# ShuangXieIrene/ssds.pytorch

Measured on AMD Instinct MI355X. Metric: images/sec (fwd+decode+NMS) SSD-MobileNetV2@512, higher is better.
Workload: dtype bf16

## Files before the change

### ssds.pytorch_amd/csrc/ssdk_mbflow.hip

```cpp
#include <stdio.h>
#include <atomic>
#include <type_traits>

#include "ssdk_common.h"
#include "ssdk_flow_common.h"

namespace ssdk {

constexpr int kFlowThreads = 256;

template <int NCH, int NFO>
struct FlowLds {
  static constexpr int T = (NCH + 1) / 2;
  static constexpr int we = 0;
  static constexpr int sb = we + NCH * 1024;
  static constexpr int wd = sb + NCH * 4 * 32;
  static constexpr int bd = wd + NCH * 9 * 4 * 8;
  static constexpr int wp = (bd + NCH * 4 * 8 + 15) & ~15;
  static constexpr int spb = wp + NFO * T * 1024;
  static constexpr int bytes = spb + NFO * 4 * 32;
};

template <int DT, int S, int NCH, int NFO, int NS, bool STEM = false, bool YE = false, bool PAIR = false, bool XD = false>
__global__ __launch_bounds__(kFlowThreads, ((STEM && !YE) || PAIR) ? 3 : 2) void mbflow_kernel(const FlowParams p) {
// ... 383 lines not shown
              db[s][3] = 0u;
            }
          }
#pragma unroll
          for (int f = 0; f < NFO; ++f) {
            const u32x4 wf = *reinterpret_cast<const u32x4*>(smem + L::wp + ((f * T + t) * 64 + (int)lane) * 16);
#pragma unroll
            for (int s = 0; s < NA; ++s) yacc[s][f] = fl_mfma<SSDK_F16>(wf, db[s], yacc[s][f]);
          }
        }
#pragma unroll
        for (int s = 0; s < NA; ++s) {
          if (out_lane[s]) {
            u16* yrow = p.y + (((size_t)n * p.Ho + oy_fin) * p.Wo + oxl[s]) * Cout;
#pragma unroll
            for (int f = 0; f < NFO; ++f) {
              const int co = f * 16 + (int)fg * 4;
              if (co < Cout) {
                const f32x4 spv = *reinterpret_cast<const f32x4*>(smem + L::spb + (f * 4 + (int)fg) * 32);
                const f32x4 bpv = *reinterpret_cast<const f32x4*>(smem + L::spb + (f * 4 + (int)fg) * 32 + 16);
                u32 h01 = fl_pack2<DT>(fmaf(yacc[s][f][0], spv[0], bpv[0]), fmaf(yacc[s][f][1], spv[1], bpv[1]));
                u32 h23 = fl_pack2<DT>(fmaf(yacc[s][f][2], spv[2], bpv[2]), fmaf(yacc[s][f][3], spv[3], bpv[3]));
                if (!STEM && !MERGE && p.residual) {
                  const u32 x01 = resv[s][f].x, x23 = resv[s][f].y;
                  h01 = fl_pack2<DT>(fl_from16<DT>(h01 & 0xffffu) + fl_from16<DT>(x01 & 0xffffu), fl_from16<DT>(h01 >> 16) + fl_from16<DT>(x01 >> 16));
                  h23 = fl_pack2<DT>(fl_from16<DT>(h23 & 0xffffu) + fl_from16<DT>(x23 & 0xffffu), fl_from16<DT>(h23 >> 16) + fl_from16<DT>(x23 >> 16));
                }
                *reinterpret_cast<uint2*>(yrow + co) = make_uint2(h01, h23);
              }
            }
          }
        }
      }
    }
    if (dbgw && dbg_k < 250) p.dbg[dbg_k++] = __builtin_readcyclecounter();
  };


  auto row2 = [&](const XRow (&x0)[NS], const XRow (&x1)[NS], int iy, fl_h2 (&a0)[NA][NCH * 2], fl_h2 (&a1)[NA][NCH * 2],
                  fl_h2 (&a2)[NA][NCH * 2], fl_h2 (&a3)[NA][NCH * 2]) {
    if (dbgw && dbg_k < 250) {
      p.dbg[dbg_k++] = __builtin_readcyclecounter();
      asm volatile("s_waitcnt vmcnt(4)" ::: "memory");
      p.dbg[dbg_k++] = __builtin_readcyclecounter();
    }
    u32x4 xf[2][NS];
    fl_f2 hi[2][NS];
#pragma unroll
    for (int s = 0; s < NS; ++s) {
#pragma unroll
      for (int q = 0; q < 4; ++q) {
        xf[0][s][q] = x0[s].w[q];
        xf[1][s][q] = x1[s].w[q];
      }
      const float k0 = (col_ok[s] && (unsigned)iy < (unsigned)p.H) ? kFlSixth : 0.f;
      const float k1 = (col_ok[s] && (unsigned)(iy + 1) < (unsigned)p.H) ? kFlSixth : 0.f;
      hi[0][s] = fl_f2{k0, k0};
      hi[1][s] = fl_f2{k1, k1};
    }
    const bool st[2] = {iy - 1 >= oy0 && iy - 1 <= oy1, iy >= oy0 && iy <= oy1};
    uint2 resv[2][NA][NFO];
    if (p.residual) {
#pragma unroll
      for (int o = 0; o < 2; ++o)
#pragma unroll
        for (int s = 0; s < NA; ++s)
#pragma unroll
          for (int f = 0; f < NFO; ++f) {
            const int co = f * 16 + (int)fg * 4;
            uint2 r = make_uint2(0u, 0u);
            if (st[o] && out_lane[s] && co < Cout) r = *reinterpret_cast<const uint2*>(ximg + ((size_t)(iy - 1 + o) * p.W + oxl[s]) * Cin + co);
            resv[o][s][f] = r;
          }
    }
    asm volatile("" ::: "memory");
    f32x4 e_cur[2][NS], e_nxt[2][NS];
    u32x4 wa = *reinterpret_cast<const u32x4*>(smem + L::we + (int)lane * 16);
    {
      const f32x4 bv0 = *reinterpret_cast<const f32x4*>(smem + L::sb + (int)fg * 32 + 16);
#pragma unroll
      for (int o = 0; o < 2; ++o)
#pragma unroll
        for (int s = 0; s < NS; ++s) e_cur[o][s] = fl_mfma<DT>(wa, xf[o][s], bv0);
    }
    if (NCH > 1) wa = *reinterpret_cast<const u32x4*>(smem + L::we + (64 + (int)lane) * 16);
#pragma unroll
    for (int c = 0; c < NCH; ++c) {
      asm volatile("" ::: "memory");
      uint2 wt[9];
#pragma unroll
      for (int t = 0; t < 9; ++t) wt[t] = *reinterpret_cast<const uint2*>(smem + L::wd + ((c * 9 + t) * 4 + (int)fg) * 8);
      const uint2 bdi = *reinterpret_cast<const uint2*>(smem + L::bd + (c * 4 + (int)fg) * 8);
      if (c + 1 < NCH) {
        const f32x4 bvn = *reinterpret_cast<const f32x4*>(smem + L::sb + ((c + 1) * 4 + (int)fg) * 32 + 16);
#pragma unroll
        for (int o = 0; o < 2; ++o)
#pragma unroll
          for (int s = 0; s < NS; ++s) e_nxt[o][s] = fl_mfma<DT>(wa, xf[o][s], bvn);
        if (c + 2 < NCH) wa = *reinterpret_cast<const u32x4*>(smem + L::we + ((c + 2) * 64 + (int)lane) * 16);
      }
      __builtin_amdgcn_sched_barrier(0);
      auto taps = [&](int ky, fl_h2 l0, fl_h2 l1, fl_h2 c0, fl_h2 c1, fl_h2 r0, fl_h2 r1, fl_h2& q0, fl_h2& q1) {
        const uint2 w0 = wt[ky * 3], w1 = wt[ky * 3 + 1], w2 = wt[ky * 3 + 2];
        fl_h2 s0 = ky == 0 ? fl_as_h2(bdi.x) : q0, s1 = ky == 0 ? fl_as_h2(bdi.y) : q1;
        s0 = __builtin_elementwise_fma(l0, fl_as_h2(w0.x), s0);
        s1 = __builtin_elementwise_fma(l1, fl_as_h2(w0.y), s1);
        s0 = __builtin_elementwise_fma(c0, fl_as_h2(w1.x), s0);
        s1 = __builtin_elementwise_fma(c1, fl_as_h2(w1.y), s1);
        if (ky == 2) {
          s0 = fl_fma_clamp01(r0, fl_as_h2(w2.x), s0);
          s1 = fl_fma_clamp01(r1, fl_as_h2(w2.y), s1);
        } else {
          s0 = __builtin_elementwise_fma(r0, fl_as_h2(w2.x), s0);
          s1 = __builtin_elementwise_fma(r1, fl_as_h2(w2.y), s1);
        }
        asm volatile("" : "+v"(s0), "+v"(s1));
        q0 = s0;
        q1 = s1;
      };
#pragma unroll
      for (int o = 0; o < 2; ++o) {
#pragma unroll
        for (int s = 0; s < NS; ++s) {
          const f32x4 e = e_cur[o][s];
          const u32 w0 = fl_unit_pack(e[0], e[1], hi[o][s]), w1 = fl_unit_pack(e[2], e[3], hi[o][s]);
          const fl_h2 l0 = fl_as_h2(fl_from_left(w0)), l1 = fl_as_h2(fl_from_left(w1)), c0 = fl_as_h2(w0), c1 = fl_as_h2(w1);
          const fl_h2 r0 = fl_as_h2(fl_from_right(w0)), r1 = fl_as_h2(fl_from_right(w1));
          if (o == 0) {
            taps(0, l0, l1, c0, c1, r0, r1, a2[s][2 * c], a2[s][2 * c + 1]);
            taps(1, l0, l1, c0, c1, r0, r1, a1[s][2 * c], a1[s][2 * c + 1]);
            taps(2, l0, l1, c0, c1, r0, r1, a0[s][2 * c], a0[s][2 * c + 1]);
          } else {
            taps(0, l0, l1, c0, c1, r0, r1, a3[s][2 * c], a3[s][2 * c + 1]);
            taps(1, l0, l1, c0, c1, r0, r1, a2[s][2 * c], a2[s][2 * c + 1]);
            taps(2, l0, l1, c0, c1, r0, r1, a1[s][2 * c], a1[s][2 * c + 1]);
          }
        }
      }
#pragma unroll
      for (int o = 0; o < 2; ++o)
#pragma unroll
        for (int s = 0; s < NS; ++s) e_cur[o][s] = e_nxt[o][s];
      __builtin_amdgcn_sched_barrier(0);
    }
    if (dbgw && dbg_k < 250) p.dbg[dbg_k++] = __builtin_readcyclecounter();
    if (st[0] || st[1]) {
      asm volatile("" ::: "memory");
      f32x4 yacc[2][NA][NFO];
#pragma unroll
      for (int o = 0; o < 2; ++o)
#pragma unroll
        for (int s = 0; s < NA; ++s)
#pragma unroll
          for (int f = 0; f < NFO; ++f) yacc[o][s][f] = f32x4{0.f, 0.f, 0.f, 0.f};
#pragma unroll
      for (int t = 0; t < T; ++t) {
        u32x4 db[2][NA];
#pragma unroll
        for (int o = 0; o < 2; ++o)
#pragma unroll
          for (int s = 0; s < NA; ++s) {
            const fl_h2* fin = o == 0 ? a0[s] : a1[s];
            db[o][s][0] = fl_as_u32(fin[4 * t]);
            db[o][s][1] = fl_as_u32(fin[4 * t + 1]);
            if (2 * t + 1 < NCH) {
              db[o][s][2] = fl_as_u32(fin[(4 * t + 2 < NCH * 2) ? 4 * t + 2 : 0]);
              db[o][s][3] = fl_as_u32(fin[(4 * t + 3 < NCH * 2) ? 4 * t + 3 : 0]);
            } else {
              db[o][s][2] = 0u;
              db[o][s][3] = 0u;
            }
          }
#pragma unroll
        for (int f = 0; f < NFO; ++f) {
          const u32x4 wf = *reinterpret_cast<const u32x4*>(smem + L::wp + ((f * T + t) * 64 + (int)lane) * 16);
#pragma unroll
          for (int o = 0; o < 2; ++o)
#pragma unroll
            for (int s = 0; s < NA; ++s) yacc[o][s][f] = fl_mfma<SSDK_F16>(wf, db[o][s], yacc[o][s][f]);
        }
      }
#pragma unroll
      for (int f = 0; f < NFO; ++f) {
        const int co = f * 16 + (int)fg * 4;
        if (co < Cout) {
          const f32x4 spv = *reinterpret_cast<const f32x4*>(smem + L::spb + (f * 4 + (int)fg) * 32);
          const f32x4 bpv = *reinterpret_cast<const f32x4*>(smem + L::spb + (f * 4 + (int)fg) * 32 + 16);
#pragma unroll
          for (int o = 0; o < 2; ++o)
#pragma unroll
            for (int s = 0; s < NA; ++s) {
              if (!(st[o] && out_lane[s])) continue;
              u16* yrow = p.y + (((size_t)n * p.Ho + (iy - 1 + o)) * p.Wo + oxl[s]) * Cout;
              u32 h01 = fl_pack2<DT>(fmaf(yacc[o][s][f][0], spv[0], bpv[0]), fmaf(yacc[o][s][f][1], spv[1], bpv[1]));
              u32 h23 = fl_pack2<DT>(fmaf(yacc[o][s][f][2], spv[2], bpv[2]), fmaf(yacc[o][s][f][3], spv[3], bpv[3]));
              if (p.residual) {
                const u32 x01 = resv[o][s][f].x, x23 = resv[o][s][f].y;
                h01 = fl_pack2<DT>(fl_from16<DT>(h01 & 0xffffu) + fl_from16<DT>(x01 & 0xffffu), fl_from16<DT>(h01 >> 16) + fl_from16<DT>(x01 >> 16));
                h23 = fl_pack2<DT>(fl_from16<DT>(h23 & 0xffffu) + fl_from16<DT>(x23 & 0xffffu), fl_from16<DT>(h23 >> 16) + fl_from16<DT>(x23 >> 16));
              }
              *reinterpret_cast<uint2*>(yrow + co) = make_uint2(h01, h23);
            }
        }
      }
    }
    if (dbgw && dbg_k < 250) p.dbg[dbg_k++] = __builtin_readcyclecounter();
  };

  const auto Y = std::true_type{};
  const auto No = std::false_type{};
  auto load_row = [&](XRow (&dst)[NS], int iy) {
#pragma unroll
    for (int s = 0; s < NS; ++s) dst[s] = load_x(iy, s);
  };
  XRow xa[NS], xb[NS];
  {
    if constexpr (PAIR) {
      const int rend = oy1 + 1;
      XRow xc[NS], xd[NS];
      load_row(xa, oy0 - 1);
      load_row(xb, oy0);
      for (int r = oy0 - 1; r <= rend; r += 4) {
        load_row(xc, r + 2);
        load_row(xd, r + 3);
        row2(xa, xb, r, accA, accB, accC, accD);
        load_row(xa, r + 4);
        load_row(xb, r + 5);
        row2(xc, xd, r + 2, accC, accD, accA, accB);
      }
    } else if constexpr (S == 1) {
      const int rend = oy1 + 1;
      load_row(xa, oy0 - 1);
      for (int r = oy0 - 1; r <= rend; r += 6) {
        load_row(xb, r + 1);
        row(xa, r, Y, Y, Y, accA, accB, accC, r - 1);
        load_row(xa, r + 2);
        row(xb, r + 1, Y, Y, Y, accB, accC, accA, r);
        load_row(xb, r + 3);
        row(xa, r + 2, Y, Y, Y, accC, accA, accB, r + 1);
        load_row(xa, r + 4);
        row(xb, r + 3, Y, Y, Y, accA, accB, accC, r + 2);
        load_row(xb, r + 5);
        row(xa, r + 4, Y, Y, Y, accB, accC, accA, r + 3);
        load_row(xa, r + 6);
        row(xb, r + 5, Y, Y, Y, accC, accA, accB, r + 4);
      }
    } else {
      const int rend = 2 * oy1 + 1;
      load_row(xa, 2 * oy0 - 1);
      for (int r = 2 * oy0 - 1; r <= rend; r += 4) {
        load_row(xb, r + 1);
        row(xa, r, Y, No, Y, accA, accC, accB, (r - 1) / 2);
        load_row(xa, r + 2);
        row(xb, r + 1, No, Y, No, accC, accB, accC, 0);
        load_row(xb, r + 3);
        row(xa, r + 2, Y, No, Y, accB, accC, accA, (r + 1) / 2);
        load_row(xa, r + 4);
        row(xb, r + 3, No, Y, No, accC, accA, accC, 0);
      }
    }
  }
}

constexpr int kFlowNS = 2;

template <int DT, int S, int NCH, int NFO>
static void flow_launch(const FlowParams& p, unsigned grid, hipStream_t stream) {
  constexpr int lds = FlowLds<NCH, NFO>::bytes;
  if constexpr (S == 1 && NCH == 9) {
    if (p.layout == 101) {
      static const int pair = getenv("SSDK_FLOW_PAIR") ? atoi(getenv("SSDK_FLOW_PAIR")) : 1;
      if (pair) {
        (void)hipFuncSetAttribute(reinterpret_cast<const void*>(&mbflow_kernel<DT, S, NCH, NFO, 1, false, false, true>), hipFuncAttributeMaxDynamicSharedMemorySize, lds);
        hipLaunchKernelGGL((mbflow_kernel<DT, S, NCH, NFO, 1, false, false, true>), dim3(grid), dim3(kFlowThreads), lds, stream, p);
        return;
      }
      (void)hipFuncSetAttribute(reinterpret_cast<const void*>(&mbflow_kernel<DT, S, NCH, NFO, 1>), hipFuncAttributeMaxDynamicSharedMemorySize, lds);
      hipLaunchKernelGGL((mbflow_kernel<DT, S, NCH, NFO, 1>), dim3(grid), dim3(kFlowThreads), lds, stream, p);
      return;
    }
  }
  (void)hipFuncSetAttribute(reinterpret_cast<const void*>(&mbflow_kernel<DT, S, NCH, NFO, kFlowNS>), hipFuncAttributeMaxDynamicSharedMemorySize, lds);
  hipLaunchKernelGGL((mbflow_kernel<DT, S, NCH, NFO, kFlowNS>), dim3(grid), dim3(kFlowThreads), lds, stream, p);
}

template <int DT, int S>
static bool flow_dispatch(const FlowParams& p, int nch, int nfo, unsigned grid, hipStream_t stream) {
#define SSDK_FLOW(NCH_, NFO_)                                   \
  if (nch == NCH_ && nfo == NFO_) {                             \
    flow_launch<DT, S, NCH_, NFO_>(p, grid, stream);            \
    return true;                                                \
  }
  SSDK_FLOW(6, 2)
  SSDK_FLOW(9, 2)
  SSDK_FLOW(12, 2)
  SSDK_FLOW(12, 4)
#undef SSDK_FLOW
  return false;
}

int launch_mbflow(const ssdk_mbconv_desc* d, hipStream_t stream) {
  static const int env = getenv("SSDK_MB_FLOW") ? atoi(getenv("SSDK_MB_FLOW")) : 1;
  const int variant = d->variant;
  if ((!env && variant <= 0) || variant < 0 || variant == 2 || variant == 3) return 1;
  const bool stem = d->stem != 0;
  if (stem) {
    if (d->Cin > 3 || d->Chid != 32 || d->Cout != 16 || d->stride != 1 || d->residual) return 1;
  } else if (d->Cin > 32 || (d->Cin % 8) || d->Chid > 192 || (d->Chid % 16) || d->Cout > 64 || (d->Cout % 8)) {
    return 1;
  }
  const int nch = d->Chid / 16, nfo = stem ? 1 : (d->Cout <= 32 ? 2 : 4);
  if (!stem && !((nch == 6 || nch == 9 || nch == 12) && (nfo == 2 || nch == 12))) return 1;
  FlowParams p;
  p.x = (const u16*)d->x;
  p.y = (u16*)d->y;
  p.we = (const u16*)d->w_expand;
  p.se = d->scale_expand;
  p.be = d->bias_expand;
  p.wd = (const u16*)d->w_dw;
  p.bd = (const u16*)d->bias_dw;
  p.wp = (const u16*)d->w_project;
  p.sp = d->scale_project;
  p.bp = d->bias_project;
  p.N = d->N;
  p.H = d->H;
  p.W = d->W;
  p.Cin = d->Cin;
  p.Himg = d->H;
  p.Wimg = d->W;
  p.Cimg = d->Cin;
  p.layout = d->stem;
  if (stem) {
    p.H = (d->H + 2 - 3) / 2 + 1;
    p.W = (d->W + 2 - 3) / 2 + 1;
    p.Cin = 32;
  }
  p.Chid = d->Chid;
  p.Cout = d->Cout;
  p.Ho = (p.H + 2 - 3) / d->stride + 1;
  p.Wo = (p.W + 2 - 3) / d->stride + 1;
  p.residual = d->residual;
  p.seg_mask = 0;
  p.dbg = nullptr;
  static const int env_dbg = getenv("SSDK_MB_DBG") ? atoi(getenv("SSDK_MB_DBG")) : 0;
  static unsigned long long* dbg_dev = nullptr;
  if (env_dbg) {
    if (!dbg_dev) (void)hipMalloc(&dbg_dev, 256 * sizeof(unsigned long long));
    (void)hipMemsetAsync(dbg_dev, 0, 256 * sizeof(unsigned long long), stream);
    p.dbg = dbg_dev;
  }
  auto dbg_print = [&]() {
    if (!env_dbg) return;
    unsigned long long hh[256];
    (void)hipStreamSynchronize(stream);
    (void)hipMemcpy(hh, dbg_dev, sizeof(hh), hipMemcpyDeviceToHost);
    fprintf(stderr, "[mbflow dbg] Cin=%d Chid=%d Cout=%d s=%d stem=%d rs=%d: per row (wait x | chunks | project+store | to next row):", d->Cin,
            d->Chid, d->Cout, d->stride, (int)stem, p.rs);
    for (int i = 0; i + 4 < 250 && hh[i + 4]; i += 4)
      fprintf(stderr, " [%llu %llu %llu %llu]", hh[i + 1] - hh[i], hh[i + 2] - hh[i + 1], hh[i + 3] - hh[i + 2], hh[i + 4] - hh[i + 3]);
    fprintf(stderr, "\n");
  };
  const int ow = d->stride == 1 ? 14 : 7;
  p.strips = (p.Wo + ow - 1) / ow;
  if (d->stride == 2) p.strips = 2 * ((p.Wo + 14) / 15);
  constexpr int env_rs = 0;
  constexpr int env_ns1 = 1;
  const bool ns1 = ((env_ns1 & 1) && !stem && d->stride == 1 && nch == 9) || ((env_ns1 & 2) && stem);
  const int flow_ns = ns1 ? 1 : kFlowNS;
  if (ns1 && !stem) p.layout = 101;
  const int groups = (p.strips + flow_ns - 1) / flow_ns;
  int rs = 64;
  while (rs > 16 && (long)d->N * groups * ((p.Ho + rs - 1) / rs) < 4096) rs >>= 1;
  if ((long)d->N * groups * ((p.Ho + rs - 1) / rs) < 2048 && env_rs <= 0 && variant <= 0) return 1;
  if (variant > 0) {
    while (rs > 8 && (long)d->N * groups * ((p.Ho + rs - 1) / rs) < 2048) rs >>= 1;
  }
  if (env_rs > 0) rs = env_rs;
  if (rs > p.Ho) rs = p.Ho;
  p.rs = rs;
  p.segs = (p.Ho + rs - 1) / rs;
  const long items = (long)d->N * groups * p.segs;
  const unsigned grid = (unsigned)((items + 3) / 4);
  bool ok;
  if (stem) {
    if (p.segs > 64) return 1;
    unsigned long long edge = 0;
    for (int sgi = 0; sgi < p.segs; ++sgi) {
      const int o0 = sgi * p.rs, o1 = (o0 + p.rs < p.Ho ? o0 + p.rs : p.Ho) - 1;
      const int last_row = o1 + 1 < p.H - 1 ? o1 + 1 : p.H - 1;
      if (2 * last_row + 1 >= p.Himg) edge |= 1ull << sgi;
    }
    const unsigned long long all = p.segs == 64 ? ~0ull : ((1ull << p.segs) - 1ull);
    constexpr int lds = FlowLds<2, 1>::bytes;
    auto go = [&](auto DTc, auto YEc, unsigned long long mask) {
      constexpr int DTv = decltype(DTc)::value;
      constexpr bool YEv = decltype(YEc)::value;
      if (!mask) return;
      FlowParams q = p;
      q.seg_mask = mask;
      const long it = (long)d->N * groups * __builtin_popcountll(mask);
      const unsigned g = (unsigned)((it + 3) / 4);
      if (ns1) {
        (void)hipFuncSetAttribute(reinterpret_cast<const void*>(&mbflow_kernel<DTv, 1, 2, 1, 1, true, YEv>),
                                  hipFuncAttributeMaxDynamicSharedMemorySize, lds);
        hipLaunchKernelGGL((mbflow_kernel<DTv, 1, 2, 1, 1, true, YEv>), dim3(g), dim3(kFlowThreads), lds, stream, q);
        return;
      }
      if constexpr (!YEv) {
        static const int env_xd = getenv("SSDK_STEM_DWORD") ? atoi(getenv("SSDK_STEM_DWORD")) : 1;
        if (env_xd && q.layout == 1 && (q.Wimg & 1) == 0 && (reinterpret_cast<uintptr_t>(q.x) & 3u) == 0) {
          (void)hipFuncSetAttribute(reinterpret_cast<const void*>(&mbflow_kernel<DTv, 1, 2, 1, kFlowNS, true, false, false, true>),
                                    hipFuncAttributeMaxDynamicSharedMemorySize, lds);
          hipLaunchKernelGGL((mbflow_kernel<DTv, 1, 2, 1, kFlowNS, true, false, false, true>), dim3(g), dim3(kFlowThreads), lds, stream, q);
          return;
        }
      }
      (void)hipFuncSetAttribute(reinterpret_cast<const void*>(&mbflow_kernel<DTv, 1, 2, 1, kFlowNS, true, YEv>),
                                hipFuncAttributeMaxDynamicSharedMemorySize, lds);
      hipLaunchKernelGGL((mbflow_kernel<DTv, 1, 2, 1, kFlowNS, true, YEv>), dim3(g), dim3(kFlowThreads), lds, stream, q);
    };
    if (d->dtype == SSDK_BF16) {
      go(std::integral_constant<int, SSDK_BF16>{}, std::false_type{}, all & ~edge);
      go(std::integral_constant<int, SSDK_BF16>{}, std::true_type{}, edge);
    } else {
      go(std::integral_constant<int, SSDK_F16>{}, std::false_type{}, all & ~edge);
      go(std::integral_constant<int, SSDK_F16>{}, std::true_type{}, edge);
    }
    dbg_print();
    return 0;
  }
  if (d->dtype == SSDK_BF16) ok = d->stride == 1 ? flow_dispatch<SSDK_BF16, 1>(p, nch, nfo, grid, stream) : flow_dispatch<SSDK_BF16, 2>(p, nch, nfo, grid, stream);
  else ok = d->stride == 1 ? flow_dispatch<SSDK_F16, 1>(p, nch, nfo, grid, stream) : flow_dispatch<SSDK_F16, 2>(p, nch, nfo, grid, stream);
  if (ok) dbg_print();
  return ok ? 0 : 1;
}

}
```

### ssds.pytorch_amd/csrc/ssdk_mbk.hip

```cpp
#include "ssdk_common.h"
#include "ssdk_flow_common.h"
#include "ssdk_scan.h"

namespace ssdk {

struct MbkParams {
  const u16* x;
  u16* y;
  const unsigned char* img;
  int N, H, W, Ho, Wo, Cin, Chid, Cout, residual;
  int pairs, halves;
  unsigned items;
  unsigned long long* dbg;
  unsigned wave_mask, pair_mask;
};

template <int KS, int NW, int NCHW, int NFO>
struct MbkGeo {
  static constexpr int NP = (NCHW + 1) / 2;
  static constexpr int PAIR_KB = 2 * KS + NFO;
  static constexpr int MISC_KB = (NCHW * 384 + 1023) / 1024;
  static constexpr int m_be = 0, m_wd = NCHW * 64, m_bd = NCHW * (64 + 288);
  static constexpr int SPB_KB = 2;
  static_assert(NFO * 128 <= SPB_KB * 1024, "projection BN block");
  __host__ __device__ static size_t weights(int halves) { return (size_t)halves * NW * NP * PAIR_KB * 1024; }
  __host__ __device__ static size_t misc_off(int halves) { return weights(halves); }
  __host__ __device__ static size_t spb_off(int halves) { return misc_off(halves) + (size_t)NW * MISC_KB * 1024; }
  __host__ __device__ static size_t bytes(int halves) { return spb_off(halves) + (size_t)halves * SPB_KB * 1024; }
};

template <int S, int NS>
struct MbkItem {
  static constexpr int NXS = NS * S;
  static constexpr int NR = S + 3;
};

template <int S, int NS, int KS, int NW, int NCHW, int NFO>
struct MbkLds {
  using G = MbkGeo<KS, NW, NCHW, NFO>;
  using I = MbkItem<S, NS>;
  static constexpr int FT = 2 * NS * NFO;
  static constexpr int XF = FT % 5 == 0 ? 5 : (FT % 8 == 0 ? 8 : 4);
  static_assert(FT % XF == 0, "exchange rounds");
  static constexpr int xt = 0;
  static constexpr int misc = xt + I::NR * I::NXS * KS * 1024;
  static constexpr int spb = misc + NW * G::MISC_KB * 1024;
  static constexpr int xch = spb + G::SPB_KB * 1024;
  static constexpr int bytes = xch + NW * XF * 1024;
};

__device__ __forceinline__ void mbk_mfma_guard() {
  __builtin_amdgcn_sched_barrier(0);
  asm volatile("s_nop 15\n\ts_nop 3" ::: "memory");
  __builtin_amdgcn_sched_barrier(0);
}
__device__ __forceinline__ void mbk_valu_guard() {
  __builtin_amdgcn_sched_barrier(0);
  asm volatile("s_nop 3" ::: "memory");
  __builtin_amdgcn_sched_barrier(0);
}
__device__ __forceinline__ u32 fl_from_left2(u32 cur, u32 prev) {
  const int old = __builtin_amdgcn_update_dpp(0, (int)prev, 0x121, 0xf, 0xf, true);
  return (u32)__builtin_amdgcn_update_dpp(old, (int)cur, 0x111, 0xf, 0xf, false);
}
__device__ __forceinline__ u32 fl_from_right2(u32 cur, u32 next) {
  const int old = __builtin_amdgcn_update_dpp(0, (int)next, 0x12f, 0xf, 0xf, true);
  return (u32)__builtin_amdgcn_update_dpp(old, (int)cur, 0x101, 0xf, 0xf, false);
}

template <int DT, int S, int NS, int KS, int NW, int NCHW, int NFO, bool DBG = false>
__global__ __launch_bounds__(64 * NW, 2) void mbk_kernel(const MbkParams p) {
  using L = MbkLds<S, NS, KS, NW, NCHW, NFO>;
  using G = MbkGeo<KS, NW, NCHW, NFO>;
  using I = MbkItem<S, NS>;
  constexpr int NR = I::NR, NXS = I::NXS, NE = NR * NXS;
  constexpr int XF = L::XF, FT = L::FT, NP = G::NP, PAIR_KB = G::PAIR_KB;
  constexpr int NO = 2 * NS;
  constexpr bool ODD = (NCHW & 1) != 0;
  constexpr int ROUNDS = FT / XF;
  extern __shared__ __attribute__((aligned(16))) unsigned char smem[];
  const u32 tid = threadIdx.x, lane = tid & 63u;
  const u32 fr = lane & 15u, fg = lane >> 4;
  const int wv = __builtin_amdgcn_readfirstlane((int)(tid >> 6));
  const int Cin = p.Cin, Cout = p.Cout, H = p.H, W = p.W, Ho = p.Ho, Wo = p.Wo;

  const u32 item = blockIdx.x;
  const int half = (int)(item % (u32)p.halves);
  const u32 rem = item / (u32)p.halves;
  const int n = (int)(rem / (u32)p.pairs), rp = (int)(rem % (u32)p.pairs);
  const int oy0 = 2 * rp;
  const int iy0 = S * oy0 - 1;
  const int co_base = half * 16 * NFO;
  const u16* ximg = p.x + (size_t)n * H * W * Cin;
  const bool stamp = p.dbg != nullptr && blockIdx.x == 0 && tid == 0;
  if (stamp) p.dbg[0] = __builtin_readcyclecounter();

  const u32x4* wimg = reinterpret_cast<const u32x4*>(p.img + ((size_t)(half * NW + wv) * NP) * ((size_t)PAIR_KB * 1024)) + lane;
  u32x4 wa[KS], wb[KS];
#pragma unroll
  for (int ks = 0; ks < KS; ++ks) {
    wa[ks] = wimg[(size_t)ks * 64];
    wb[ks] = wimg[(size_t)(KS + ks) * 64];
  }

  for (int e = wv; e < NE; e += NW) {
    const int r = e / NXS, xs = e % NXS;
    int iy = iy0 + r;
    iy = iy < 0 ? 0 : (iy > H - 1 ? H - 1 : iy);
    const int col = S == 1 ? 16 * xs + (int)fr : 2 * (16 * (xs >> 1) + (int)fr) + (xs & 1);
    const u16* src = ximg + ((size_t)iy * W + col) * Cin + fg * 8;
#pragma unroll
    for (int ks = 0; ks < KS; ++ks)
      __builtin_amdgcn_global_load_lds((glb_u8*)(src + ks * 32), (lds_u8*)(smem + L::xt + (e * KS + ks) * 1024), 16, 0, 0);
  }
  {
    const unsigned char* src = p.img + G::misc_off(p.halves) + (size_t)wv * (G::MISC_KB * 1024) + lane * 16;
#pragma unroll
    for (int k = 0; k < G::MISC_KB; ++k)
      __builtin_amdgcn_global_load_lds((glb_u8*)(src + k * 1024), (lds_u8*)(smem + L::misc + (wv * G::MISC_KB + k) * 1024), 16, 0, 0);
  }
  if (wv == 0) {
    const unsigned char* src = p.img + G::spb_off(p.halves) + (size_t)half * (G::SPB_KB * 1024) + lane * 16;
#pragma unroll
    for (int k = 0; k < G::SPB_KB; ++k)
      __builtin_amdgcn_global_load_lds((glb_u8*)(src + k * 1024), (lds_u8*)(smem + L::spb + k * 1024), 16, 0, 0);
  }
  asm volatile("s_waitcnt vmcnt(0)" ::: "memory");
  __syncthreads();
  if (stamp) p.dbg[1] = __builtin_readcyclecounter();

  fl_f2 hi[NR];
#pragma unroll
  for (int r = 0; r < NR; ++r) {
    const float k = ((unsigned)(iy0 + r) < (unsigned)H) ? kFlSixth : 0.f;
    hi[r] = fl_f2{k, k};
  }

  f32x4 yacc[NO][NFO];
#pragma unroll
  for (int o = 0; o < NO; ++o)
#pragma unroll
    for (int f = 0; f < NFO; ++f) yacc[o][f] = f32x4{0.f, 0.f, 0.f, 0.f};

  const unsigned char* xt = smem + L::xt + lane * 16;
  const unsigned char* mc = smem + L::misc + wv * (G::MISC_KB * 1024);

  auto chunk = [&](int c, const u32x4 (&w)[KS], u32 (&dout)[NO][2]) {
    const f32x4 bv = *reinterpret_cast<const f32x4*>(mc + G::m_be + (c * 4 + (int)fg) * 16);
    f32x4 e[NE];
#pragma unroll
    for (int i = 0; i < NE; ++i) e[i] = bv;
#pragma unroll
    for (int ks = 0; ks < KS; ++ks) {
      u32x4 xf[NE];
#pragma unroll
      for (int i = 0; i < NE; ++i) xf[i] = *reinterpret_cast<const u32x4*>(xt + (i * KS + ks) * 1024);
#pragma unroll
      for (int i = 0; i < NE; ++i) e[i] = fl_mfma<DT>(w[ks], xf[i], e[i]);
    }
    uint2 wt[9];
#pragma unroll
    for (int t = 0; t < 9; ++t) wt[t] = *reinterpret_cast<const uint2*>(mc + G::m_wd + ((c * 9 + t) * 4 + (int)fg) * 8);
    const uint2 bdi = *reinterpret_cast<const uint2*>(mc + G::m_bd + (c * 4 + (int)fg) * 8);
    mbk_mfma_guard();
    u32 ew[NR][NXS][2];
#pragma unroll
    for (int r = 0; r < NR; ++r)
#pragma unroll
      for (int xs = 0; xs < NXS; ++xs) {
        ew[r][xs][0] = fl_unit_pack(e[r * NXS + xs][0], e[r * NXS + xs][1], hi[r]);
        ew[r][xs][1] = fl_unit_pack(e[r * NXS + xs][2], e[r * NXS + xs][3], hi[r]);
      }
#pragma unroll
    for (int o = 0; o < 2; ++o)
#pragma unroll
      for (int j = 0; j < NS; ++j) {
        fl_h2 s[2] = {fl_as_h2(bdi.x), fl_as_h2(bdi.y)};
#pragma unroll
        for (int ky = 0; ky < 3; ++ky) {
          const int r = S * o + ky;
          const uint2 w0 = wt[ky * 3], w1 = wt[ky * 3 + 1], w2 = wt[ky * 3 + 2];
#pragma unroll
          for (int wd = 0; wd < 2; ++wd) {
            u32 tl, tc, tr;
            if constexpr (S == 1) {
              tc = ew[r][j][wd];
              tl = j == 0 ? fl_from_left(tc) : fl_from_left2(tc, ew[r][j > 0 ? j - 1 : 0][wd]);
              tr = j == NS - 1 ? fl_from_right(tc) : fl_from_right2(tc, ew[r][j < NS - 1 ? j + 1 : j][wd]);
            } else {
              const u32 odd = ew[r][2 * j + 1][wd];
              tc = ew[r][2 * j][wd];
              tl = j == 0 ? fl_from_left(odd) : fl_from_left2(odd, ew[r][j > 0 ? 2 * j - 1 : 1][wd]);
              tr = odd;
            }
            const u32 ww0 = wd ? w0.y : w0.x, ww1 = wd ? w1.y : w1.x, ww2 = wd ? w2.y : w2.x;
            s[wd] = __builtin_elementwise_fma(fl_as_h2(tl), fl_as_h2(ww0), s[wd]);
            s[wd] = __builtin_elementwise_fma(fl_as_h2(tc), fl_as_h2(ww1), s[wd]);
            if (ky == 2) s[wd] = fl_fma_clamp01(fl_as_h2(tr), fl_as_h2(ww2), s[wd]);
            else s[wd] = __builtin_elementwise_fma(fl_as_h2(tr), fl_as_h2(ww2), s[wd]);
          }
        }
        dout[o * NS + j][0] = fl_as_u32(s[0]);
        dout[o * NS + j][1] = fl_as_u32(s[1]);
      }
  };

  constexpr int FH = NFO / 2;
  for (int t = 0; t < NP; ++t) {
    const u32x4* wp = wimg + (size_t)t * (PAIR_KB * 64);
    const bool last = t == NP - 1;
    const u32x4* wn = wimg + (size_t)(last ? t : t + 1) * (PAIR_KB * 64);
    u32 d0[NO][2], d1[NO][2];
    u32x4 wf0[FH], wf1[NFO - FH];
#pragma unroll
    for (int f = 0; f < FH; ++f) wf0[f] = wp[(size_t)(2 * KS + f) * 64];
    chunk(2 * t, wa, d0);
    __builtin_amdgcn_sched_barrier(0);
    u32x4 na[KS];
#pragma unroll
    for (int ks = 0; ks < KS; ++ks) na[ks] = wn[(size_t)ks * 64];
#pragma unroll
    for (int f = FH; f < NFO; ++f) wf1[f - FH] = wp[(size_t)(2 * KS + f) * 64];
    if (!(ODD && last)) {
      chunk(2 * t + 1, wb, d1);
    } else {
#pragma unroll
      for (int o = 0; o < NO; ++o) d1[o][0] = d1[o][1] = 0u;
    }
    __builtin_amdgcn_sched_barrier(0);
    u32x4 nb[KS];
#pragma unroll
    for (int ks = 0; ks < KS; ++ks) nb[ks] = wn[(size_t)(KS + ks) * 64];
    u32x4 db[NO];
#pragma unroll
    for (int o = 0; o < NO; ++o) db[o] = u32x4{d0[o][0], d0[o][1], d1[o][0], d1[o][1]};
    if constexpr (DBG) {
      if (!((p.pair_mask >> t) & 1u) || !((p.wave_mask >> wv) & 1u)) {
#pragma unroll
        for (int o = 0; o < NO; ++o) db[o] = u32x4{0u, 0u, 0u, 0u};
      }
    }
    mbk_valu_guard();
#pragma unroll
    for (int f = 0; f < NFO; ++f)
#pragma unroll
      for (int o = 0; o < NO; ++o)
        yacc[o][f] = fl_mfma<SSDK_F16>(f < FH ? wf0[f < FH ? f : 0] : wf1[f >= FH ? f - FH : 0], db[o], yacc[o][f]);
    __builtin_amdgcn_sched_barrier(0);
#pragma unroll
    for (int ks = 0; ks < KS; ++ks) {
      wa[ks] = na[ks];
      wb[ks] = nb[ks];
    }
  }
  if (stamp) p.dbg[2] = __builtin_readcyclecounter();

  unsigned char* xb = smem + L::xch;
  const unsigned char* spb = smem + L::spb;
  constexpr int GPW = (XF + NW - 1) / NW;
  uint2 resv[ROUNDS][GPW];
#pragma unroll
  for (int R = 0; R < ROUNDS; ++R)
#pragma unroll
    for (int gg = 0; gg < GPW; ++gg) {
      const int g = wv + gg * NW, q = R * XF + g, oj = q / NFO, f = q % NFO;
      const int oy = oy0 + oj / NS, ox = 16 * (oj % NS) + (int)fr, co = co_base + f * 16 + (int)fg * 4;
      resv[R][gg] = make_uint2(0u, 0u);
      if (S == 1 && p.residual && g < XF && oy < Ho && co < Cout)
        resv[R][gg] = *reinterpret_cast<const uint2*>(ximg + ((size_t)oy * W + ox) * Cin + co);
    }
#pragma unroll
  for (int R = 0; R < ROUNDS; ++R) {
#pragma unroll
    for (int g = 0; g < XF; ++g) {
      const int q = R * XF + g, oj = q / NFO, f = q % NFO;
      *reinterpret_cast<f32x4*>(xb + ((wv * XF + g) * 64 + (int)lane) * 16) = yacc[oj][f];
    }
    __syncthreads();
#pragma unroll
    for (int gg = 0; gg < GPW; ++gg) {
      const int g = wv + gg * NW;
      if (g < XF) {
        const int q = R * XF + g, oj = q / NFO, f = q % NFO;
        f32x4 y = *reinterpret_cast<const f32x4*>(xb + ((0 * XF + g) * 64 + (int)lane) * 16);
#pragma unroll
        for (int w2 = 1; w2 < NW; ++w2) {
          const f32x4 t2 = *reinterpret_cast<const f32x4*>(xb + ((w2 * XF + g) * 64 + (int)lane) * 16);
          y = y + t2;
        }
        const int oy = oy0 + oj / NS, ox = 16 * (oj % NS) + (int)fr;
        const int co = co_base + f * 16 + (int)fg * 4;
        if (oy < Ho && co < Cout) {
          const f32x4 spv = *reinterpret_cast<const f32x4*>(spb + (f * 4 + (int)fg) * 32);
          const f32x4 bpv = *reinterpret_cast<const f32x4*>(spb + (f * 4 + (int)fg) * 32 + 16);
          u32 h01 = fl_pack2<DT>(fmaf(y[0], spv[0], bpv[0]), fmaf(y[1], spv[1], bpv[1]));
          u32 h23 = fl_pack2<DT>(fmaf(y[2], spv[2], bpv[2]), fmaf(y[3], spv[3], bpv[3]));
          if (S == 1 && p.residual) {
            const uint2 xr = resv[R][gg];
            h01 = fl_pack2<DT>(fl_from16<DT>(h01 & 0xffffu) + fl_from16<DT>(xr.x & 0xffffu), fl_from16<DT>(h01 >> 16) + fl_from16<DT>(xr.x >> 16));
            h23 = fl_pack2<DT>(fl_from16<DT>(h23 & 0xffffu) + fl_from16<DT>(xr.y & 0xffffu), fl_from16<DT>(h23 >> 16) + fl_from16<DT>(xr.y >> 16));
          }
          u16* yrow = p.y + (((size_t)n * Ho + oy) * Wo + ox) * Cout;
          *reinterpret_cast<uint2*>(yrow + co) = make_uint2(h01, h23);
        }
      }
    }
    if (R + 1 < ROUNDS) __syncthreads();
  }
  if (stamp) p.dbg[3] = __builtin_readcyclecounter();
}

template <int DT, int S, int NS, int KS, int NW, int NCHW, int NFO, bool DBG = false>
static void mbk_launch(const MbkParams& p, hipStream_t stream) {
  constexpr int lds = MbkLds<S, NS, KS, NW, NCHW, NFO>::bytes;
  static_assert(lds <= 160 * 1024, "LDS");
  (void)hipFuncSetAttribute(reinterpret_cast<const void*>(&mbk_kernel<DT, S, NS, KS, NW, NCHW, NFO, DBG>),
                            hipFuncAttributeMaxDynamicSharedMemorySize, lds);
  hipLaunchKernelGGL((mbk_kernel<DT, S, NS, KS, NW, NCHW, NFO, DBG>), dim3(p.items), dim3(64 * NW), lds, stream, p);
}

constexpr int kMbkNW = 4;
struct MbkInst {
  int s, ns, ks, nchw, nfo;
};
static const MbkInst kMbkInst[] = {{1, 1, 5, 15, 10}, {2, 1, 3, 9, 10}, {1, 2, 2, 6, 4}, {1, 2, 2, 6, 6}, {1, 2, 3, 9, 6},
                                   {2, 2, 1, 3, 4}, {1, 4, 1, 3, 2}};

static int mbk_find(int stride, int Wo, int Cin, int Chid, int Cout, int nw, int* halves) {
  if (nw != kMbkNW || Cin % 32 || Chid % 16 || Cout % 16 || Wo % 16) return -1;
  const int ks = Cin / 32, nch = Chid / 16, nchw = (nch + nw - 1) / nw, ns = Wo / 16;
  for (int i = 0; i < (int)(sizeof(kMbkInst) / sizeof(kMbkInst[0])); ++i) {
    const MbkInst& k = kMbkInst[i];
    if (k.s == stride && k.ns == ns && k.ks == ks && k.nchw == nchw && Cout % (16 * k.nfo) == 0) {
      if (halves) *halves = Cout / (16 * k.nfo);
      return i;
    }
  }
  return -1;
}

static size_t mbk_bytes(int inst, int halves) {
  switch (inst) {
    case 0: return MbkGeo<5, kMbkNW, 15, 10>::bytes(halves);
    case 1: return MbkGeo<3, kMbkNW, 9, 10>::bytes(halves);
    case 2: return MbkGeo<2, kMbkNW, 6, 4>::bytes(halves);
    case 3: return MbkGeo<2, kMbkNW, 6, 6>::bytes(halves);
    case 4: return MbkGeo<3, kMbkNW, 9, 6>::bytes(halves);
    case 5: return MbkGeo<1, kMbkNW, 3, 4>::bytes(halves);
    case 6: return MbkGeo<1, kMbkNW, 3, 2>::bytes(halves);
  }
  return 0;
}

template <int DT>
static void mbk_dispatch(const MbkParams& p, int inst, hipStream_t stream) {
  const bool dbg = p.wave_mask != ~0u || p.pair_mask != ~0u;
  switch (inst) {
    case 0: dbg ? mbk_launch<DT, 1, 1, 5, kMbkNW, 15, 10, true>(p, stream) : mbk_launch<DT, 1, 1, 5, kMbkNW, 15, 10>(p, stream); break;
    case 1: mbk_launch<DT, 2, 1, 3, kMbkNW, 9, 10>(p, stream); break;
    case 2: mbk_launch<DT, 1, 2, 2, kMbkNW, 6, 4>(p, stream); break;
    case 3: mbk_launch<DT, 1, 2, 2, kMbkNW, 6, 6>(p, stream); break;
    case 4: mbk_launch<DT, 1, 2, 3, kMbkNW, 9, 6>(p, stream); break;
    case 5: mbk_launch<DT, 2, 2, 1, kMbkNW, 3, 4>(p, stream); break;
    case 6: mbk_launch<DT, 1, 4, 1, kMbkNW, 3, 2>(p, stream); break;
  }
}

int launch_mbk(const ssdk_mbconv_desc* d, hipStream_t stream) {
  static const int env = getenv("SSDK_MBK") ? atoi(getenv("SSDK_MBK")) : 1;
  const int variant = d->variant;
  if ((!env && variant != 3) || (variant != 0 && variant != 3)) return 1;
  if (d->stem || !d->w_image || d->image_nw < 1 || (d->stride != 1 && d->stride != 2)) return 1;
  const int Ho = (d->H + 2 - 3) / d->stride + 1, Wo = (d->W + 2 - 3) / d->stride + 1;
  if (d->W != Wo * d->stride) return 1;
  int halves = 0;
  const int inst = mbk_find(d->stride, Wo, d->Cin, d->Chid, d->Cout, d->image_nw, &halves);
  if (inst < 0 || (size_t)d->w_image_bytes < mbk_bytes(inst, halves) || ((uintptr_t)d->w_image & 15)) return 1;
  if (env != 1 && variant != 3 && !((env >> (inst + 1)) & 1)) return 1;
  const int pairs = (Ho + 1) / 2;
  const long items = (long)halves * d->N * pairs;
  constexpr int env_min = 256;
  if (items < env_min && variant != 3) return 1;
  MbkParams p;
  p.x = (const u16*)d->x;
  p.y = (u16*)d->y;
  p.img = (const unsigned char*)d->w_image;
  p.N = d->N;
  p.H = d->H;
  p.W = d->W;
  p.Ho = Ho;
  p.Wo = Wo;
  p.Cin = d->Cin;
  p.Chid = d->Chid;
  p.Cout = d->Cout;
  p.residual = d->residual;
  p.pairs = pairs;
  p.halves = halves;
  p.items = (unsigned)items;
  p.dbg = nullptr;
  p.wave_mask = p.pair_mask = ~0u;
  if (const char* m = getenv("SSDK_MBK_MASKS")) {
    unsigned a = ~0u, b = ~0u;
    if (sscanf(m, "%x,%x", &a, &b) == 2) {
      p.wave_mask = a;
      p.pair_mask = b;
    }
  }
  static const int env_dbg = getenv("SSDK_MB_DBG") ? atoi(getenv("SSDK_MB_DBG")) : 0;
  static unsigned long long* dbg_dev = nullptr;
  if (env_dbg) {
    if (!dbg_dev) (void)hipMalloc(&dbg_dev, 8 * sizeof(unsigned long long));
    p.dbg = dbg_dev;
  }
  if (d->dtype == SSDK_BF16) mbk_dispatch<SSDK_BF16>(p, inst, stream);
  else mbk_dispatch<SSDK_F16>(p, inst, stream);
  if (env_dbg) {
    unsigned long long h[4];
    (void)hipStreamSynchronize(stream);
    (void)hipMemcpy(h, dbg_dev, sizeof(h), hipMemcpyDeviceToHost);
    fprintf(stderr, "[mbk dbg] Cin=%d Chid=%d Cout=%d s=%d W=%d items=%ld : setup %llu loop %llu exchange %llu\n", d->Cin, d->Chid,
            d->Cout, d->stride, d->W, items, h[1] - h[0], h[2] - h[1], h[3] - h[2]);
  }
  return 0;
}

}

extern "C" size_t ssdk_mbk_image_bytes(int Cin, int Chid, int Cout, int stride, int Wo, int nw, int* nfo) {
  int halves = 0;
  const int inst = ssdk::mbk_find(stride, Wo, Cin, Chid, Cout, nw, &halves);
  if (inst < 0) return 0;
  if (nfo) *nfo = ssdk::kMbkInst[inst].nfo;
  return ssdk::mbk_bytes(inst, halves);
}
```

Before: 64510.

## Software-pipeline mbk expand/depthwise/project across chunk pairs with scheduled interleaving

Adds a pipelined path to the fused MBConv kernel. The expand MFMAs of the next chunk and the projection MFMAs of the previous pair are overlapped with the VALU depthwise work of the current chunk, and sched_group_barrier hints interleave the two. This path becomes the default for instances 0, 2 and 3, with variant 4 selecting the old serial path. The pack and clamp helpers move to local inline asm, and the row-validity scale becomes wave-uniform through readfirstlane. The cost is higher register pressure, plus a risk of hazards in the hand-tuned scheduling.

```diff
diff --git a/ssds.pytorch_amd/csrc/ssdk_mbflow.hip b/ssds.pytorch_amd/csrc/ssdk_mbflow.hip
--- a/ssds.pytorch_amd/csrc/ssdk_mbflow.hip
+++ b/ssds.pytorch_amd/csrc/ssdk_mbflow.hip
@@ -709,7 +709,7 @@
 int launch_mbflow(const ssdk_mbconv_desc* d, hipStream_t stream) {
   static const int env = getenv("SSDK_MB_FLOW") ? atoi(getenv("SSDK_MB_FLOW")) : 1;
   const int variant = d->variant;
-  if ((!env && variant <= 0) || variant < 0 || variant == 2 || variant == 3) return 1;
+  if ((!env && variant <= 0) || variant < 0 || variant == 2 || variant == 3 || variant == 4) return 1;
   const bool stem = d->stem != 0;
   if (stem) {
     if (d->Cin > 3 || d->Chid != 32 || d->Cout != 16 || d->stride != 1 || d->residual) return 1;
diff --git a/ssds.pytorch_amd/csrc/ssdk_mbk.hip b/ssds.pytorch_amd/csrc/ssdk_mbk.hip
--- a/ssds.pytorch_amd/csrc/ssdk_mbk.hip
+++ b/ssds.pytorch_amd/csrc/ssdk_mbk.hip
@@ -59,6 +59,38 @@
   asm volatile("s_nop 3" ::: "memory");
   __builtin_amdgcn_sched_barrier(0);
 }
+template <bool B>
+struct MbkFlag {
+  static constexpr bool value = B;
+};
+template <int NX, int NJ, int DV>
+__device__ __forceinline__ void mbk_interleave() {
+  if constexpr (NX + NJ > 0) {
+    constexpr int V = DV / (NX + NJ) > 0 ? DV / (NX + NJ) : 1;
+    if constexpr (NX > 0) __builtin_amdgcn_sched_group_barrier(0x100, 2, 0);
+#pragma unroll
+    for (int m = 0; m < NX; ++m) {
+      __builtin_amdgcn_sched_group_barrier(0x8, 1, 0);
+      __builtin_amdgcn_sched_group_barrier(0x100, 1, 0);
+      __builtin_amdgcn_sched_group_barrier(0x2, V, 0);
+    }
+#pragma unroll
+    for (int m = 0; m < NJ; ++m) {
+      __builtin_amdgcn_sched_group_barrier(0x8, 1, 0);
+      __builtin_amdgcn_sched_group_barrier(0x2, V, 0);
+    }
+  }
+}
+__device__ __forceinline__ u32 mbk_unit_pack(float a, float b, fl_f2 k) {
+  const fl_f2 v = {a, b};
+  fl_f2 r;
+  asm("v_pk_mul_f32 %0, %1, %2 clamp" : "=v"(r) : "v"(v), "s"(k));
+  return __builtin_bit_cast(u32, __builtin_amdgcn_cvt_pkrtz(r[0], r[1]));
+}
+__device__ __forceinline__ fl_h2 mbk_fma_clamp01(fl_h2 a, fl_h2 b, fl_h2 c) {
+  asm("v_pk_fma_f16 %0, %1, %2, %0 clamp" : "+v"(c) : "v"(a), "v"(b));
+  return c;
+}
 __device__ __forceinline__ u32 fl_from_left2(u32 cur, u32 prev) {
   const int old = __builtin_amdgcn_update_dpp(0, (int)prev, 0x121, 0xf, 0xf, true);
   return (u32)__builtin_amdgcn_update_dpp(old, (int)cur, 0x111, 0xf, 0xf, false);
@@ -68,7 +100,7 @@
   return (u32)__builtin_amdgcn_update_dpp(old, (int)cur, 0x101, 0xf, 0xf, false);
 }
 
-template <int DT, int S, int NS, int KS, int NW, int NCHW, int NFO, bool DBG = false>
+template <int DT, int S, int NS, int KS, int NW, int NCHW, int NFO, bool DBG = false, bool PIPE = false>
 __global__ __launch_bounds__(64 * NW, 2) void mbk_kernel(const MbkParams p) {
   using L = MbkLds<S, NS, KS, NW, NCHW, NFO>;
   using G = MbkGeo<KS, NW, NCHW, NFO>;
@@ -132,7 +164,8 @@
   fl_f2 hi[NR];
 #pragma unroll
   for (int r = 0; r < NR; ++r) {
-    const float k = ((unsigned)(iy0 + r) < (unsigned)H) ? kFlSixth : 0.f;
+    const int kb = __builtin_amdgcn_readfirstlane(((unsigned)(iy0 + r) < (unsigned)H) ? __builtin_bit_cast(int, kFlSixth) : 0);
+    const float k = __builtin_bit_cast(float, kb);
     hi[r] = fl_f2{k, k};
   }
 
@@ -145,32 +178,23 @@
   const unsigned char* xt = smem + L::xt + lane * 16;
   const unsigned char* mc = smem + L::misc + wv * (G::MISC_KB * 1024);
 
-  auto chunk = [&](int c, const u32x4 (&w)[KS], u32 (&dout)[NO][2]) {
-    const f32x4 bv = *reinterpret_cast<const f32x4*>(mc + G::m_be + (c * 4 + (int)fg) * 16);
-    f32x4 e[NE];
-#pragma unroll
-    for (int i = 0; i < NE; ++i) e[i] = bv;
-#pragma unroll
-    for (int ks = 0; ks < KS; ++ks) {
-      u32x4 xf[NE];
-#pragma unroll
-      for (int i = 0; i < NE; ++i) xf[i] = *reinterpret_cast<const u32x4*>(xt + (i * KS + ks) * 1024);
-#pragma unroll
-      for (int i = 0; i < NE; ++i) e[i] = fl_mfma<DT>(w[ks], xf[i], e[i]);
-    }
-    uint2 wt[9];
+  auto bias_of = [&](int c) __attribute__((always_inline)) { return *reinterpret_cast<const f32x4*>(mc + G::m_be + (c * 4 + (int)fg) * 16); };
+  auto taps_of = [&](int c, uint2 (&wt)[9], uint2& bdi) __attribute__((always_inline)) {
 #pragma unroll
     for (int t = 0; t < 9; ++t) wt[t] = *reinterpret_cast<const uint2*>(mc + G::m_wd + ((c * 9 + t) * 4 + (int)fg) * 8);
-    const uint2 bdi = *reinterpret_cast<const uint2*>(mc + G::m_bd + (c * 4 + (int)fg) * 8);
+    bdi = *reinterpret_cast<const uint2*>(mc + G::m_bd + (c * 4 + (int)fg) * 8);
+  };
+  auto pack = [&](const f32x4 (&e)[NE], u32 (&ew)[NR][NXS][2]) __attribute__((always_inline)) {
     mbk_mfma_guard();
-    u32 ew[NR][NXS][2];
 #pragma unroll
     for (int r = 0; r < NR; ++r)
 #pragma unroll
       for (int xs = 0; xs < NXS; ++xs) {
-        ew[r][xs][0] = fl_unit_pack(e[r * NXS + xs][0], e[r * NXS + xs][1], hi[r]);
-        ew[r][xs][1] = fl_unit_pack(e[r * NXS + xs][2], e[r * NXS + xs][3], hi[r]);
-      }
+        ew[r][xs][0] = mbk_unit_pack(e[r * NXS + xs][0], e[r * NXS + xs][1], hi[r]);
+        ew[r][xs][1] = mbk_unit_pack(e[r * NXS + xs][2], e[r * NXS + xs][3], hi[r]);
+      }
+  };
+  auto depthwise = [&](const u32 (&ew)[NR][NXS][2], const uint2 (&wt)[9], const uint2 bdi, u32 (&dout)[NO][2]) __attribute__((always_inline)) {
 #pragma unroll
     for (int o = 0; o < 2; ++o)
 #pragma unroll
@@ -196,7 +220,7 @@
             const u32 ww0 = wd ? w0.y : w0.x, ww1 = wd ? w1.y : w1.x, ww2 = wd ? w2.y : w2.x;
             s[wd] = __builtin_elementwise_fma(fl_as_h2(tl), fl_as_h2(ww0), s[wd]);
             s[wd] = __builtin_elementwise_fma(fl_as_h2(tc), fl_as_h2(ww1), s[wd]);
-            if (ky == 2) s[wd] = fl_fma_clamp01(fl_as_h2(tr), fl_as_h2(ww2), s[wd]);
+            if (ky == 2) s[wd] = mbk_fma_clamp01(fl_as_h2(tr), fl_as_h2(ww2), s[wd]);
             else s[wd] = __builtin_elementwise_fma(fl_as_h2(tr), fl_as_h2(ww2), s[wd]);
           }
         }
@@ -204,8 +228,28 @@
         dout[o * NS + j][1] = fl_as_u32(s[1]);
       }
   };
+  auto chunk = [&](int c, const u32x4 (&w)[KS], u32 (&dout)[NO][2]) __attribute__((always_inline)) {
+    const f32x4 bv = bias_of(c);
+    f32x4 e[NE];
+#pragma unroll
+    for (int i = 0; i < NE; ++i) e[i] = bv;
+#pragma unroll
+    for (int ks = 0; ks < KS; ++ks) {
+      u32x4 xf[NE];
+#pragma unroll
+      for (int i = 0; i < NE; ++i) xf[i] = *reinterpret_cast<const u32x4*>(xt + (i * KS + ks) * 1024);
+#pragma unroll
+      for (int i = 0; i < NE; ++i) e[i] = fl_mfma<DT>(w[ks], xf[i], e[i]);
+    }
+    uint2 wt[9], bdi;
+    taps_of(c, wt, bdi);
+    u32 ew[NR][NXS][2];
+    pack(e, ew);
+    depthwise(ew, wt, bdi, dout);
+  };
 
   constexpr int FH = NFO / 2;
+  if constexpr (!PIPE) {
   for (int t = 0; t < NP; ++t) {
     const u32x4* wp = wimg + (size_t)t * (PAIR_KB * 64);
     const bool last = t == NP - 1;
@@ -252,6 +296,120 @@
       wa[ks] = na[ks];
       wb[ks] = nb[ks];
     }
+  }
+  } else {
+    static_assert(NP >= 2, "the pipeline's first and last pair are two pairs");
+    constexpr int FP = FH + NO / 4;
+    constexpr int DV = NO * (S == 1 ? (NS == 1 ? 28 : 34) : 25);
+    f32x4 e[NE];
+    u32x4 dbp[NO];
+    u32x4 wf0[FP], wf1[NFO - FP];
+    u32x4 wl[NFO];
+    auto expand = [&](const u32x4 (&w)[KS], const f32x4 bv, f32x4 (&ee)[NE]) __attribute__((always_inline)) {
+#pragma unroll
+      for (int i = 0; i < NE; ++i) ee[i] = bv;
+#pragma unroll
+      for (int ks = 0; ks < KS; ++ks)
+#pragma unroll
+        for (int i = 0; i < NE; ++i) {
+          const u32x4 xf = *reinterpret_cast<const u32x4*>(xt + (i * KS + ks) * 1024);
+          ee[i] = fl_mfma<DT>(w[ks], xf, ee[i]);
+        }
+    };
+    auto project = [&](const u32x4* wf, const int f0, const int nf, const u32x4 (&db)[NO]) __attribute__((always_inline)) {
+#pragma unroll
+      for (int f = 0; f < nf; ++f)
+#pragma unroll
+        for (int o = 0; o < NO; ++o) yacc[o][f0 + f] = fl_mfma<SSDK_F16>(wf[f], db[o], yacc[o][f0 + f]);
+    };
+    auto pair = [&](auto first_, auto last_, const int t) __attribute__((always_inline)) {
+      constexpr bool FIRST = decltype(first_)::value, LAST = decltype(last_)::value;
+      constexpr bool HAS1 = !(ODD && LAST);
+      const u32x4* wp = wimg + (size_t)t * (PAIR_KB * 64);
+      const u32x4* wn = wp + PAIR_KB * 64;
+      const u32x4* wq = wp - PAIR_KB * 64;
+      u32 d0[NO][2], d1[NO][2];
+      if constexpr (!LAST) {
+#pragma unroll
+        for (int ks = 0; ks < KS; ++ks) wa[ks] = wn[(size_t)ks * 64];
+      } else if constexpr (!HAS1) {
+#pragma unroll
+        for (int f = 0; f < NFO; ++f) wl[f] = wp[(size_t)(2 * KS + f) * 64];
+      }
+      if constexpr (!FIRST) {
+#pragma unroll
+        for (int f = 0; f < FP; ++f) wf0[f] = wq[(size_t)(2 * KS + f) * 64];
+        if constexpr (!HAS1) {
+#pragma unroll
+          for (int f = FP; f < NFO; ++f) wf1[f - FP] = wq[(size_t)(2 * KS + f) * 64];
+        }
+      }
+      {
+        constexpr int NX = HAS1 ? NE * KS : 0, NJ = FIRST ? 0 : NO * (HAS1 ? FP : NFO);
+        uint2 wt[9], bdi;
+        taps_of(2 * t, wt, bdi);
+        f32x4 bv = {0.f, 0.f, 0.f, 0.f};
+        if constexpr (HAS1) bv = bias_of(2 * t + 1);
+        u32 ew[NR][NXS][2];
+        pack(e, ew);
+        __builtin_amdgcn_sched_barrier(0);
+        if constexpr (HAS1) expand(wb, bv, e);
+        if constexpr (!FIRST) {
+          project(wf0, 0, FP, dbp);
+          if constexpr (!HAS1) project(wf1, FP, NFO - FP, dbp);
+        }
+        depthwise(ew, wt, bdi, d0);
+        mbk_interleave<NX, NJ, DV>();
+        __builtin_amdgcn_sched_barrier(0);
+      }
+      mbk_valu_guard();
+      if constexpr (LAST && HAS1) {
+#pragma unroll
+        for (int f = 0; f < NFO; ++f) wl[f] = wp[(size_t)(2 * KS + f) * 64];
+      }
+      if constexpr (HAS1) {
+        constexpr int NX = LAST ? 0 : NE * KS, NJ = FIRST ? 0 : NO * (NFO - FP);
+        if constexpr (!LAST) {
+#pragma unroll
+          for (int ks = 0; ks < KS; ++ks) wb[ks] = wn[(size_t)(KS + ks) * 64];
+        }
+        if constexpr (!FIRST) {
+#pragma unroll
+          for (int f = FP; f < NFO; ++f) wf1[f - FP] = wq[(size_t)(2 * KS + f) * 64];
+        }
+        uint2 wt[9], bdi;
+        taps_of(2 * t + 1, wt, bdi);
+        f32x4 bv = {0.f, 0.f, 0.f, 0.f};
+        if constexpr (!LAST) bv = bias_of(2 * t + 2);
+        u32 ew[NR][NXS][2];
+        pack(e, ew);
+        __builtin_amdgcn_sched_barrier(0);
+        if constexpr (!LAST) expand(wa, bv, e);
+        if constexpr (!FIRST) project(wf1, FP, NFO - FP, dbp);
+        depthwise(ew, wt, bdi, d1);
+        mbk_interleave<NX, NJ, DV>();
+        __builtin_amdgcn_sched_barrier(0);
+        mbk_valu_guard();
+      } else {
+#pragma unroll
+        for (int o = 0; o < NO; ++o) d1[o][0] = d1[o][1] = 0u;
+      }
+#pragma unroll
+      for (int o = 0; o < NO; ++o) dbp[o] = u32x4{d0[o][0], d0[o][1], d1[o][0], d1[o][1]};
+      if constexpr (DBG) {
+        if (!((p.pair_mask >> t) & 1u) || !((p.wave_mask >> wv) & 1u)) {
+#pragma unroll
+          for (int o = 0; o < NO; ++o) dbp[o] = u32x4{0u, 0u, 0u, 0u};
+        }
+      }
+    };
+    expand(wa, bias_of(0), e);
+    pair(MbkFlag<true>{}, MbkFlag<false>{}, 0);
+#pragma nounroll
+    for (int t = 1; t < NP - 1; ++t) pair(MbkFlag<false>{}, MbkFlag<false>{}, t);
+    pair(MbkFlag<false>{}, MbkFlag<true>{}, NP - 1);
+    mbk_valu_guard();
+    project(wl, 0, NFO, dbp);
   }
   if (stamp) p.dbg[2] = __builtin_readcyclecounter();
 
@@ -310,13 +468,13 @@
   if (stamp) p.dbg[3] = __builtin_readcyclecounter();
 }
 
-template <int DT, int S, int NS, int KS, int NW, int NCHW, int NFO, bool DBG = false>
+template <int DT, int S, int NS, int KS, int NW, int NCHW, int NFO, bool DBG = false, bool PIPE = false>
 static void mbk_launch(const MbkParams& p, hipStream_t stream) {
   constexpr int lds = MbkLds<S, NS, KS, NW, NCHW, NFO>::bytes;
   static_assert(lds <= 160 * 1024, "LDS");
-  (void)hipFuncSetAttribute(reinterpret_cast<const void*>(&mbk_kernel<DT, S, NS, KS, NW, NCHW, NFO, DBG>),
+  (void)hipFuncSetAttribute(reinterpret_cast<const void*>(&mbk_kernel<DT, S, NS, KS, NW, NCHW, NFO, DBG, PIPE>),
                             hipFuncAttributeMaxDynamicSharedMemorySize, lds);
-  hipLaunchKernelGGL((mbk_kernel<DT, S, NS, KS, NW, NCHW, NFO, DBG>), dim3(p.items), dim3(64 * NW), lds, stream, p);
+  hipLaunchKernelGGL((mbk_kernel<DT, S, NS, KS, NW, NCHW, NFO, DBG, PIPE>), dim3(p.items), dim3(64 * NW), lds, stream, p);
 }
 
 constexpr int kMbkNW = 4;
@@ -352,14 +510,14 @@
   return 0;
 }
 
-template <int DT>
+template <int DT, bool PIPE>
 static void mbk_dispatch(const MbkParams& p, int inst, hipStream_t stream) {
   const bool dbg = p.wave_mask != ~0u || p.pair_mask != ~0u;
   switch (inst) {
-    case 0: dbg ? mbk_launch<DT, 1, 1, 5, kMbkNW, 15, 10, true>(p, stream) : mbk_launch<DT, 1, 1, 5, kMbkNW, 15, 10>(p, stream); break;
+    case 0: dbg ? mbk_launch<DT, 1, 1, 5, kMbkNW, 15, 10, true, PIPE>(p, stream) : mbk_launch<DT, 1, 1, 5, kMbkNW, 15, 10, false, PIPE>(p, stream); break;
     case 1: mbk_launch<DT, 2, 1, 3, kMbkNW, 9, 10>(p, stream); break;
-    case 2: mbk_launch<DT, 1, 2, 2, kMbkNW, 6, 4>(p, stream); break;
-    case 3: mbk_launch<DT, 1, 2, 2, kMbkNW, 6, 6>(p, stream); break;
+    case 2: mbk_launch<DT, 1, 2, 2, kMbkNW, 6, 4, false, PIPE>(p, stream); break;
+    case 3: mbk_launch<DT, 1, 2, 2, kMbkNW, 6, 6, false, PIPE>(p, stream); break;
     case 4: mbk_launch<DT, 1, 2, 3, kMbkNW, 9, 6>(p, stream); break;
     case 5: mbk_launch<DT, 2, 2, 1, kMbkNW, 3, 4>(p, stream); break;
     case 6: mbk_launch<DT, 1, 4, 1, kMbkNW, 3, 2>(p, stream); break;
@@ -368,7 +526,8 @@
 
 int launch_mbk(const ssdk_mbconv_desc* d, hipStream_t stream) {
   static const int env = getenv("SSDK_MBK") ? atoi(getenv("SSDK_MBK")) : 1;
-  const int variant = d->variant;
+  const int variant = d->variant == 4 ? 3 : d->variant;
+  const bool serial = d->variant == 4;
   if ((!env && variant != 3) || (variant != 0 && variant != 3)) return 1;
   if (d->stem || !d->w_image || d->image_nw < 1 || (d->stride != 1 && d->stride != 2)) return 1;
   const int Ho = (d->H + 2 - 3) / d->stride + 1, Wo = (d->W + 2 - 3) / d->stride + 1;
@@ -412,8 +571,8 @@
     if (!dbg_dev) (void)hipMalloc(&dbg_dev, 8 * sizeof(unsigned long long));
     p.dbg = dbg_dev;
   }
-  if (d->dtype == SSDK_BF16) mbk_dispatch<SSDK_BF16>(p, inst, stream);
-  else mbk_dispatch<SSDK_F16>(p, inst, stream);
+  if (d->dtype == SSDK_BF16) serial ? mbk_dispatch<SSDK_BF16, false>(p, inst, stream) : mbk_dispatch<SSDK_BF16, true>(p, inst, stream);
+  else serial ? mbk_dispatch<SSDK_F16, false>(p, inst, stream) : mbk_dispatch<SSDK_F16, true>(p, inst, stream);
   if (env_dbg) {
     unsigned long long h[4];
     (void)hipStreamSynchronize(stream);
```

Result: no change. 64610, median of 2 (+0.2%).
